# ieellee/uLLSAM

Measured on AMD Instinct MI355X. Metric: images/s end-to-end (ViT+LLM+mask) 1024^2, higher is better.
Workload: dtype bf16; 1 GPU; uLLSAM mask path (app.py:580-645): SAM ViT-H + InternLM2-7b-shaped prefill S=1081 + prompt encoder + mask decoder + x4 upsample/threshold, 1 point prompt/image, batch 4/GPU; batch_per_gpu=4, global_batch=4, seq_len=1081, vit_linears=bf16

## Files before the change

### ullsam_amd/csrc/norm.hip

```cpp
#include "common.h"

struct NormArgs {
    const void* in;
    void* out;
    const float* w;
    const float* b;
    long rows;
    int D;
    long in_stride, out_stride;
    float eps;
    int rms;
    int act;
    const float* post_scale;
    const float* post_shift;
};

template <typename TI, typename TO, int MAXV>
__global__ __launch_bounds__(256) void norm_kernel(NormArgs p) {
    const int lane = threadIdx.x & 63;
    const long row = (long)blockIdx.x * 4 + (threadIdx.x >> 6);
    if (row >= p.rows) return;
    const TI* x = reinterpret_cast<const TI*>(p.in) + row * p.in_stride;
    TO* y = reinterpret_cast<TO*>(p.out) + row * p.out_stride;
    const int nv = p.D >> 2;
    float4 v[MAXV];
    float s = 0.f;
#pragma unroll
    for (int i = 0; i < MAXV; ++i) {
        const int idx = i * 64 + lane;
        if (idx < nv) {
            v[i] = load4(x + idx * 4);
            s += (v[i].x + v[i].y) + (v[i].z + v[i].w);
        } else {
            v[i] = make_float4(0.f, 0.f, 0.f, 0.f);
        }
    }
    float mean = 0.f;
    if (!p.rms) mean = wave_sum(s) / (float)p.D;
    float ss = 0.f;
#pragma unroll
    for (int i = 0; i < MAXV; ++i) {
        const int idx = i * 64 + lane;
        if (idx < nv) {
            const float a = v[i].x - mean, b = v[i].y - mean, c = v[i].z - mean, d = v[i].w - mean;
            ss += (a * a + b * b) + (c * c + d * d);
        }
    }
    const float var = wave_sum(ss) / (float)p.D;
    const float rstd = p.rms ? rsqrtf(var + p.eps) : 1.0f / sqrtf(var + p.eps);
    const float ps = p.post_scale ? p.post_scale[0] : 1.f;
    const float pb = p.post_shift ? p.post_shift[0] : 0.f;
    const bool post = p.post_scale || p.post_shift;
#pragma unroll
    for (int i = 0; i < MAXV; ++i) {
        const int idx = i * 64 + lane;
        if (idx < nv) {
            float4 o = make_float4((v[i].x - mean) * rstd, (v[i].y - mean) * rstd, (v[i].z - mean) * rstd, (v[i].w - mean) * rstd);
            if (p.w) {
                const float4 w = *reinterpret_cast<const float4*>(p.w + idx * 4);
                o.x *= w.x; o.y *= w.y; o.z *= w.z; o.w *= w.w;
            }
            if (p.b) {
                const float4 b = *reinterpret_cast<const float4*>(p.b + idx * 4);
                o.x += b.x; o.y += b.y; o.z += b.z; o.w += b.w;
            }
            if (post) { o.x = o.x * ps + pb; o.y = o.y * ps + pb; o.z = o.z * ps + pb; o.w = o.w * ps + pb; }
            if (p.act == 1) { o.x = gelu_erf(o.x); o.y = gelu_erf(o.y); o.z = gelu_erf(o.z); o.w = gelu_erf(o.w); }
            store4(y + idx * 4, o);
        }
    }
}

template <typename TI, typename TO, int MAXV, int WPR = 4>
__global__ __launch_bounds__(256) void norm_block_kernel(NormArgs p) {
    __shared__ float red[2][4];
    constexpr int TPR = WPR * 64;
    const int tid = threadIdx.x, lane = tid & 63, wv = tid >> 6;
    const int sub = wv / WPR, t = tid - sub * TPR;
    const long row = (long)blockIdx.x * (4 / WPR) + sub;
    const bool live = row < p.rows;
    const TI* x = reinterpret_cast<const TI*>(p.in) + (live ? row : 0) * p.in_stride;
    TO* y = reinterpret_cast<TO*>(p.out) + (live ? row : 0) * p.out_stride;
    const int nv = p.D >> 2;
    float4 v[MAXV];
    float s = 0.f;
#pragma unroll
    for (int i = 0; i < MAXV; ++i) {
        const int idx = i * TPR + t;
        if (idx < nv && live) {
            v[i] = load4(x + idx * 4);
            s += (v[i].x + v[i].y) + (v[i].z + v[i].w);
        } else {
            v[i] = make_float4(0.f, 0.f, 0.f, 0.f);
        }
    }
    auto row_sum = [&](float part, int slot) -> float {
        part = wave_sum(part);
        if (lane == 0) red[slot][wv] = part;
        __syncthreads();
        float tot = red[slot][sub * WPR];
#pragma unroll
        for (int k = 1; k < WPR; ++k) tot += red[slot][sub * WPR + k];
        return tot;
    };
    float mean = 0.f;
    if (!p.rms) mean = row_sum(s, 0) / (float)p.D;
    float ss = 0.f;
#pragma unroll
    for (int i = 0; i < MAXV; ++i) {
        const int idx = i * TPR + t;
        if (idx < nv && live) {
            const float a = v[i].x - mean, b = v[i].y - mean, c = v[i].z - mean, d = v[i].w - mean;
            ss += (a * a + b * b) + (c * c + d * d);
        }
    }
    const float var = row_sum(ss, 1) / (float)p.D;
    const float rstd = p.rms ? rsqrtf(var + p.eps) : 1.0f / sqrtf(var + p.eps);
    const float ps = p.post_scale ? p.post_scale[0] : 1.f;
    const float pb = p.post_shift ? p.post_shift[0] : 0.f;
    const bool post = p.post_scale || p.post_shift;
    if (!live) return;
#pragma unroll
    for (int i = 0; i < MAXV; ++i) {
        const int idx = i * TPR + t;
        if (idx < nv) {
            float4 o = make_float4((v[i].x - mean) * rstd, (v[i].y - mean) * rstd, (v[i].z - mean) * rstd, (v[i].w - mean) * rstd);
            if (p.w) {
                const float4 w = *reinterpret_cast<const float4*>(p.w + idx * 4);
                o.x *= w.x; o.y *= w.y; o.z *= w.z; o.w *= w.w;
            }
            if (p.b) {
                const float4 b = *reinterpret_cast<const float4*>(p.b + idx * 4);
                o.x += b.x; o.y += b.y; o.z += b.z; o.w += b.w;
            }
            if (post) { o.x = o.x * ps + pb; o.y = o.y * ps + pb; o.z = o.z * ps + pb; o.w = o.w * ps + pb; }
            if (p.act == 1) { o.x = gelu_erf(o.x); o.y = gelu_erf(o.y); o.z = gelu_erf(o.z); o.w = gelu_erf(o.w); }
            store4(y + idx * 4, o);
        }
    }
}

template <typename TI, typename TO>
__global__ __launch_bounds__(256) void norm_narrow_kernel(NormArgs p) {
    const int lane = threadIdx.x & 63, sub = lane & 15;
    const long row = ((long)blockIdx.x * 4 + (threadIdx.x >> 6)) * 4 + (lane >> 4);
    const int nv = p.D >> 2;
    const bool on = row < p.rows && sub < nv;
    const TI* x = reinterpret_cast<const TI*>(p.in) + (on ? row : 0) * p.in_stride;
    float4 v = make_float4(0.f, 0.f, 0.f, 0.f);
    if (on) v = load4(x + sub * 4);
    float s = (v.x + v.y) + (v.z + v.w);
    float mean = 0.f;
    if (!p.rms) {
        for (int o = 8; o > 0; o >>= 1) s += __shfl_xor(s, o, 64);
        mean = s / (float)p.D;
    }
    float ss = 0.f;
    if (on) {
        const float a = v.x - mean, b = v.y - mean, c = v.z - mean, d = v.w - mean;
        ss = (a * a + b * b) + (c * c + d * d);
    }
    for (int o = 8; o > 0; o >>= 1) ss += __shfl_xor(ss, o, 64);
    const float var = ss / (float)p.D;
    const float rstd = p.rms ? rsqrtf(var + p.eps) : 1.0f / sqrtf(var + p.eps);
    if (!on) return;
    float4 o = make_float4((v.x - mean) * rstd, (v.y - mean) * rstd, (v.z - mean) * rstd, (v.w - mean) * rstd);
    if (p.w) {
        const float4 w = *reinterpret_cast<const float4*>(p.w + sub * 4);
        o.x *= w.x; o.y *= w.y; o.z *= w.z; o.w *= w.w;
    }
    if (p.b) {
        const float4 b = *reinterpret_cast<const float4*>(p.b + sub * 4);
        o.x += b.x; o.y += b.y; o.z += b.z; o.w += b.w;
    }
    if (p.post_scale || p.post_shift) {
        const float ps = p.post_scale ? p.post_scale[0] : 1.f, pb = p.post_shift ? p.post_shift[0] : 0.f;
        o.x = o.x * ps + pb; o.y = o.y * ps + pb; o.z = o.z * ps + pb; o.w = o.w * ps + pb;
    }
    if (p.act == 1) { o.x = gelu_erf(o.x); o.y = gelu_erf(o.y); o.z = gelu_erf(o.z); o.w = gelu_erf(o.w); }
    store4(reinterpret_cast<TO*>(p.out) + row * p.out_stride + sub * 4, o);
}

static int g_norm_lds = 0;
extern "C" int ullsam_set_norm_variant(int v) { g_norm_lds = v; return 0; }

template <typename TI, typename TO>
static int launch_norm(const NormArgs& a, hipStream_t s) {
    const dim3 grid((unsigned)((a.rows + 3) / 4)), block(256);
    const int nv = a.D / 4;
    if (nv <= 16 && a.rows >= 4096) {
        norm_narrow_kernel<TI, TO><<<dim3((unsigned)((a.rows + 15) / 16)), block, 0, s>>>(a);
        ULLSAM_LAUNCH_CHECK();
        return 0;
    }
    if (g_norm_lds == 0 && (a.rows >= 1024 || a.rows <= 64) && nv >= 512) {
        const dim3 g((unsigned)a.rows);
        if (nv <= 512) norm_block_kernel<TI, TO, 2><<<g, block, 0, s>>>(a);
        else norm_block_kernel<TI, TO, 4><<<g, block, 0, s>>>(a);
        ULLSAM_LAUNCH_CHECK();
        return 0;
    }
    const size_t lds = 0;
    if (nv <= 64) norm_kernel<TI, TO, 1><<<grid, block, lds, s>>>(a);
    else if (nv <= 256) norm_kernel<TI, TO, 4><<<grid, block, lds, s>>>(a);
    else if (nv <= 512) norm_kernel<TI, TO, 8><<<grid, block, lds, s>>>(a);
    else norm_kernel<TI, TO, 16><<<grid, block, lds, s>>>(a);
    ULLSAM_LAUNCH_CHECK();
    return 0;
}

template <typename TO>
__global__ __launch_bounds__(256) void norm_fanout_kernel(const float* __restrict__ in, long rows, int D, const float* __restrict__ w,
                                                          const float* __restrict__ b, float eps, float* __restrict__ out_f32,
                                                          TO* __restrict__ out_c, TO* __restrict__ out_c_pe,
                                                          const float* __restrict__ pe, long pe_rows) {
    const int lane = threadIdx.x & 63;
    const long row = (long)blockIdx.x * 4 + (threadIdx.x >> 6);
    if (row >= rows) return;
    const int nv = D >> 2;
    const bool on = lane < nv;
    float4 v = make_float4(0.f, 0.f, 0.f, 0.f);
    if (on) v = *reinterpret_cast<const float4*>(in + row * D + lane * 4);
    const float mean = wave_sum((v.x + v.y) + (v.z + v.w)) / (float)D;
    float ss = 0.f;
    if (on) {
        const float a = v.x - mean, bb = v.y - mean, c = v.z - mean, d = v.w - mean;
        ss = (a * a + bb * bb) + (c * c + d * d);
    }
    const float rstd = 1.0f / sqrtf(wave_sum(ss) / (float)D + eps);
    if (!on) return;
    float4 o = make_float4((v.x - mean) * rstd, (v.y - mean) * rstd, (v.z - mean) * rstd, (v.w - mean) * rstd);
    if (w) { const float4 t = *reinterpret_cast<const float4*>(w + lane * 4); o.x *= t.x; o.y *= t.y; o.z *= t.z; o.w *= t.w; }
    if (b) { const float4 t = *reinterpret_cast<const float4*>(b + lane * 4); o.x += t.x; o.y += t.y; o.z += t.z; o.w += t.w; }
    if (out_f32) *reinterpret_cast<float4*>(out_f32 + row * D + lane * 4) = o;
    if (out_c) store4(out_c + row * D + lane * 4, o);
    if (out_c_pe) {
        const float4 t = *reinterpret_cast<const float4*>(pe + (row % pe_rows) * D + lane * 4);
        store4(out_c_pe + row * D + lane * 4, make_float4(o.x + t.x, o.y + t.y, o.z + t.z, o.w + t.w));
    }
}

extern "C" int ullsam_norm_fanout(const float* in, long rows, int D, const float* w, const float* b, float eps, float* out_f32,
                                  void* out_c, void* out_c_pe, int c_dtype, const float* pe, long pe_rows, void* stream) {
    ULLSAM_CHECK(D % 4 == 0 && D > 0 && D <= 256, "norm_fanout: D=%d must be a multiple of 4 and <= 256", D);
    ULLSAM_CHECK(!out_c_pe || (pe && pe_rows > 0), "norm_fanout: out_c_pe needs pe");
    if (rows <= 0) return 0;
    hipStream_t s = reinterpret_cast<hipStream_t>(stream);
    const dim3 grid((unsigned)((rows + 3) / 4));
    if (c_dtype == 0) norm_fanout_kernel<float><<<grid, 256, 0, s>>>(in, rows, D, w, b, eps, out_f32, (float*)out_c, (float*)out_c_pe, pe, pe_rows);
    else norm_fanout_kernel<bf16><<<grid, 256, 0, s>>>(in, rows, D, w, b, eps, out_f32, (bf16*)out_c, (bf16*)out_c_pe, pe, pe_rows);
    ULLSAM_LAUNCH_CHECK();
    return 0;
}

extern "C" int ullsam_norm(const void* in, int in_dtype, long in_stride, void* out, int out_dtype, long out_stride,
                           const float* w, const float* b, long rows, int D, float eps, int rms, int act,
                           const float* post_scale, const float* post_shift, void* stream) {
    ULLSAM_CHECK(D % 4 == 0 && D > 0 && D <= 4096, "ullsam_norm: D=%d must be a multiple of 4 and <= 4096", D);
    ULLSAM_CHECK(rows >= 0, "ullsam_norm: bad rows");
    if (rows == 0) return 0;
    ULLSAM_CHECK(in_stride % 4 == 0 && out_stride % 4 == 0, "ullsam_norm: strides must be multiples of 4 elements");
    NormArgs a{in, out, w, rms ? nullptr : b, rows, D, in_stride, out_stride, eps, rms, act, post_scale, post_shift};
    hipStream_t s = reinterpret_cast<hipStream_t>(stream);
    if (in_dtype == 0 && out_dtype == 0) return launch_norm<float, float>(a, s);
    if (in_dtype == 0 && out_dtype == 1) return launch_norm<float, bf16>(a, s);
    if (in_dtype == 1 && out_dtype == 1) return launch_norm<bf16, bf16>(a, s);
    if (in_dtype == 1 && out_dtype == 0) return launch_norm<bf16, float>(a, s);
    ULLSAM_CHECK(false, "ullsam_norm: bad dtypes %d %d", in_dtype, out_dtype);
}

template <typename TI, int MAXV>
__global__ __launch_bounds__(256) void rows_fp8_kernel(const TI* __restrict__ in, long in_stride, unsigned char* __restrict__ out, long out_stride,
                                                      float* __restrict__ scale, const float* __restrict__ w, const float* __restrict__ b, long rows, int D,
                                                      float eps, int do_norm) {
    const int lane = threadIdx.x & 63;
    const long row = (long)blockIdx.x * 4 + (threadIdx.x >> 6);
    if (row >= rows) return;
    const TI* x = in + row * in_stride;
    const int nv = D >> 2;
    float4 v[MAXV];
    float s = 0.f;
#pragma unroll
    for (int i = 0; i < MAXV; ++i) {
        const int idx = i * 64 + lane;
        v[i] = idx < nv ? load4(x + idx * 4) : make_float4(0.f, 0.f, 0.f, 0.f);
        s += (v[i].x + v[i].y) + (v[i].z + v[i].w);
    }
    if (do_norm) {
        const float mean = wave_sum(s) / (float)D;
        float ss = 0.f;
#pragma unroll
        for (int i = 0; i < MAXV; ++i)
            if (i * 64 + lane < nv) {
                const float a = v[i].x - mean, bb = v[i].y - mean, c = v[i].z - mean, d = v[i].w - mean;
                ss += (a * a + bb * bb) + (c * c + d * d);
            }
        const float rstd = 1.0f / sqrtf(wave_sum(ss) / (float)D + eps);
#pragma unroll
        for (int i = 0; i < MAXV; ++i) {
            const int idx = i * 64 + lane;
            if (idx < nv) {
                const float4 g = *reinterpret_cast<const float4*>(w + idx * 4), be = *reinterpret_cast<const float4*>(b + idx * 4);
                v[i].x = (v[i].x - mean) * rstd * g.x + be.x; v[i].y = (v[i].y - mean) * rstd * g.y + be.y;
                v[i].z = (v[i].z - mean) * rstd * g.z + be.z; v[i].w = (v[i].w - mean) * rstd * g.w + be.w;
            }
        }
    }
    float amax = 0.f;
#pragma unroll
    for (int i = 0; i < MAXV; ++i) amax = fmaxf(amax, fmaxf(fmaxf(fabsf(v[i].x), fabsf(v[i].y)), fmaxf(fabsf(v[i].z), fabsf(v[i].w))));
    amax = wave_max(amax);
    const float sc = amax > 0.f ? amax * (1.0f / 448.0f) : 1.0f;
    const float inv = 1.0f / sc;
    if (lane == 0) scale[row] = sc;
    unsigned int* y = reinterpret_cast<unsigned int*>(out + row * out_stride);
#pragma unroll
    for (int i = 0; i < MAXV; ++i) {
        const int idx = i * 64 + lane;
        if (idx < nv) {
            const float q0 = fminf(fmaxf(v[i].x * inv, -448.f), 448.f), q1 = fminf(fmaxf(v[i].y * inv, -448.f), 448.f);
            const float q2 = fminf(fmaxf(v[i].z * inv, -448.f), 448.f), q3 = fminf(fmaxf(v[i].w * inv, -448.f), 448.f);
            int pk = __builtin_amdgcn_cvt_pk_fp8_f32(q0, q1, 0, false);
            pk = __builtin_amdgcn_cvt_pk_fp8_f32(q2, q3, pk, true);
            y[idx] = (unsigned int)pk;
        }
    }
}

extern "C" int ullsam_rows_fp8(const void* in, int in_dtype, long in_stride, void* out, long out_stride, float* scale, const float* w,
                               const float* b, long rows, int D, float eps, void* stream) {
    ULLSAM_CHECK(D % 4 == 0 && D <= 8192 && rows >= 0, "ullsam_rows_fp8: D=%d must be a multiple of 4, <= 8192", D);
    ULLSAM_CHECK((w == nullptr) == (b == nullptr), "ullsam_rows_fp8: weight and bias go together");
    ULLSAM_CHECK(out_stride % 4 == 0 && ((uintptr_t)out & 3) == 0, "ullsam_rows_fp8: output rows must be 4-byte aligned");
    if (rows == 0) return 0;
    hipStream_t s = reinterpret_cast<hipStream_t>(stream);
    const dim3 grid((unsigned)((rows + 3) / 4));
    const int nv = D / 4, maxv = (nv + 63) / 64;
    const int dn = w != nullptr;
#define ULLSAM_RF8(TI, MV) rows_fp8_kernel<TI, MV><<<grid, 256, 0, s>>>(reinterpret_cast<const TI*>(in), in_stride, reinterpret_cast<unsigned char*>(out), out_stride, scale, w, b, rows, D, eps, dn)
    if (in_dtype == ULLSAM_DT_F32) {
        if (maxv <= 4) ULLSAM_RF8(float, 4); else if (maxv <= 8) ULLSAM_RF8(float, 8); else if (maxv <= 16) ULLSAM_RF8(float, 16); else ULLSAM_RF8(float, 32);
    } else {
        if (maxv <= 4) ULLSAM_RF8(bf16, 4); else if (maxv <= 8) ULLSAM_RF8(bf16, 8); else if (maxv <= 16) ULLSAM_RF8(bf16, 16); else ULLSAM_RF8(bf16, 32);
    }
#undef ULLSAM_RF8
    ULLSAM_LAUNCH_CHECK();
    return 0;
}

template <typename TI>
__global__ __launch_bounds__(256) void rows_fp8_pow2_kernel(const TI* __restrict__ in, long in_stride, unsigned char* __restrict__ out, long out_stride,
                                                           float* __restrict__ scale, long rows, int D) {
    const int lane = threadIdx.x & 63;
    const long row = (long)blockIdx.x * 4 + (threadIdx.x >> 6);
    if (row >= rows) return;
    const TI* x = in + row * in_stride;
    const int nv = D >> 2;
    float amax = 0.f;
    for (int idx = lane; idx < nv; idx += 64) {
        const float4 v = load4(x + idx * 4);
        amax = fmaxf(amax, fmaxf(fmaxf(fabsf(v.x), fabsf(v.y)), fmaxf(fabsf(v.z), fabsf(v.w))));
    }
    amax = wave_max(amax);
    float sc = 1.0f, inv = 1.0f;
    if (amax > 0.f) {
        int e;
        const float f = frexpf(amax, &e);
        const int s = max((f <= 0.875f ? e - 9 : e - 8), -126);
        sc = ldexpf(1.0f, s);
        inv = ldexpf(1.0f, -s);
    }
    if (lane == 0) scale[row] = sc;
    unsigned int* y = reinterpret_cast<unsigned int*>(out + row * out_stride);
    for (int idx = lane; idx < nv; idx += 64) {
        const float4 v = load4(x + idx * 4);
        const float q0 = fminf(fmaxf(v.x * inv, -448.f), 448.f), q1 = fminf(fmaxf(v.y * inv, -448.f), 448.f);
        const float q2 = fminf(fmaxf(v.z * inv, -448.f), 448.f), q3 = fminf(fmaxf(v.w * inv, -448.f), 448.f);
        int pk = __builtin_amdgcn_cvt_pk_fp8_f32(q0, q1, 0, false);
        pk = __builtin_amdgcn_cvt_pk_fp8_f32(q2, q3, pk, true);
        y[idx] = (unsigned int)pk;
    }
}

extern "C" int ullsam_rows_fp8_pow2(const void* in, int in_dtype, long in_stride, void* out, long out_stride, float* scale, long rows, int D,
                                    void* stream) {
    ULLSAM_CHECK(in_dtype == ULLSAM_DT_F32 || in_dtype == ULLSAM_DT_BF16, "ullsam_rows_fp8_pow2: bad dtype %d", in_dtype);
    ULLSAM_CHECK(D > 0 && D % 4 == 0 && rows >= 0 && rows <= 4l * 0x7fffffff, "ullsam_rows_fp8_pow2: D=%d must be a positive multiple of 4", D);
    ULLSAM_CHECK(in_stride >= D && in_stride % 4 == 0 && ((uintptr_t)in & (in_dtype == ULLSAM_DT_F32 ? 15 : 7)) == 0, "ullsam_rows_fp8_pow2: input rows must be aligned groups of 4 elements");
    ULLSAM_CHECK(out_stride >= D && out_stride % 4 == 0 && ((uintptr_t)out & 3) == 0, "ullsam_rows_fp8_pow2: output rows must be 4-byte aligned");
    ULLSAM_CHECK(in && out && scale, "ullsam_rows_fp8_pow2: null argument");
    if (rows == 0) return 0;
    hipStream_t s = reinterpret_cast<hipStream_t>(stream);
    const dim3 grid((unsigned)((rows + 3) / 4));
    if (in_dtype == ULLSAM_DT_F32) rows_fp8_pow2_kernel<float><<<grid, 256, 0, s>>>(reinterpret_cast<const float*>(in), in_stride, reinterpret_cast<unsigned char*>(out), out_stride, scale, rows, D);
    else rows_fp8_pow2_kernel<bf16><<<grid, 256, 0, s>>>(reinterpret_cast<const bf16*>(in), in_stride, reinterpret_cast<unsigned char*>(out), out_stride, scale, rows, D);
    ULLSAM_LAUNCH_CHECK();
    return 0;
}
```

Baseline: 54.03 images/s.

## Add persistent double-buffered streaming layernorm kernel for fp32-to-bf16 rows

Adds a persistent grid-stride norm kernel for fp32-in, bf16-out rows at common widths (1280, 2048, 3072, 4096). It keeps weights and bias in registers, prefetches the next row while reducing the current one, and pairs lanes with DPP swaps to issue 16-byte stores. The grid is capped at a few workgroups per CU. The goal is to hide load latency and cut launch and tail overhead for the ViT and LLM norms, at the cost of more register use, a changed reduction order, and new variant-flag encoding.

```diff
diff --git a/ullsam_amd/csrc/norm.hip b/ullsam_amd/csrc/norm.hip
--- a/ullsam_amd/csrc/norm.hip
+++ b/ullsam_amd/csrc/norm.hip
@@ -1,4 +1,5 @@
 #include "common.h"
+#include <type_traits>
 
 struct NormArgs {
     const void* in;
@@ -181,19 +182,164 @@
     store4(reinterpret_cast<TO*>(p.out) + row * p.out_stride + sub * 4, o);
 }
 
-static int g_norm_lds = 0;
-extern "C" int ullsam_set_norm_variant(int v) { g_norm_lds = v; return 0; }
+typedef unsigned int u32x4 __attribute__((ext_vector_type(4)));
+
+template <bool NT> __device__ __forceinline__ f32x4 load_row4(const float* p) {
+    if (NT) return __builtin_nontemporal_load(reinterpret_cast<const f32x4*>(p));
+    return *reinterpret_cast<const f32x4*>(p);
+}
+__device__ __forceinline__ float centred_sumsq(f32x4 v, float mean) {
+#pragma clang fp contract(off)
+    const float a = v.x - mean, b = v.y - mean, c = v.z - mean, d = v.w - mean;
+    return __builtin_fmaf(a, a, b * b) + __builtin_fmaf(c, c, d * d);
+}
+__device__ __forceinline__ uint2v norm_affine_bf16(f32x4 v, float mean, float rstd, float4 w, float4 b, bool has_w, bool has_b) {
+#pragma clang fp contract(off)
+    float4 o = make_float4((v.x - mean) * rstd, (v.y - mean) * rstd, (v.z - mean) * rstd, (v.w - mean) * rstd);
+    if (has_w) { o.x *= w.x; o.y *= w.y; o.z *= w.z; o.w *= w.w; }
+    if (has_b) { o.x += b.x; o.y += b.y; o.z += b.z; o.w += b.w; }
+    bf16x4_t h;
+    h[0] = (bf16)o.x; h[1] = (bf16)o.y; h[2] = (bf16)o.z; h[3] = (bf16)o.w;
+    return __builtin_bit_cast(uint2v, h);
+}
+__device__ __forceinline__ unsigned int lane_xor1(unsigned int v) { return (unsigned int)__builtin_amdgcn_mov_dpp((int)v, 0xB1, 0xF, 0xF, true); }
+
+template <int NV, int WPR, bool NT>
+__global__ __launch_bounds__(256) void norm_stream_kernel(NormArgs p) {
+    __shared__ float red[4][4];
+    constexpr int TPR = WPR * 64;
+    const int tid = threadIdx.x, lane = tid & 63, wv = tid >> 6;
+    const int t = WPR == 1 ? lane : tid;
+    long row = WPR == 1 ? (long)blockIdx.x * 4 + __builtin_amdgcn_readfirstlane(wv) : (long)blockIdx.x;
+    const long stride = WPR == 1 ? (long)gridDim.x * 4 : (long)gridDim.x;
+    const float* xin = reinterpret_cast<const float*>(p.in);
+    bf16* yout = reinterpret_cast<bf16*>(p.out);
+    const bool has_w = p.w != nullptr, has_b = p.b != nullptr;
+    float4 w[NV], b[NV];
+#pragma unroll
+    for (int i = 0; i < NV; ++i) {
+        w[i] = has_w ? *reinterpret_cast<const float4*>(p.w + (i * TPR + t) * 4) : make_float4(0.f, 0.f, 0.f, 0.f);
+        b[i] = has_b ? *reinterpret_cast<const float4*>(p.b + (i * TPR + t) * 4) : make_float4(0.f, 0.f, 0.f, 0.f);
+    }
+    auto row_sum = [&](float part, int slot) -> float {
+        part = wave_sum(part);
+        if (WPR == 1) return part;
+        if (lane == 0) red[slot][wv] = part;
+        __syncthreads();
+        float tot = red[slot][0];
+#pragma unroll
+        for (int k = 1; k < 4; ++k) tot += red[slot][k];
+        return tot;
+    };
+    if (row >= p.rows) return;
+    auto issue = [&](f32x4 (&v)[NV], long r, int spread) {
+        const float* x = xin + r * p.in_stride;
+#pragma unroll
+        for (int i = 0; i < NV; ++i) v[i] = load_row4<NT>(x + (i * TPR + t) * 4 * spread);
+    };
+    int left = (int)((p.rows - row + stride - 1) / stride);
+    auto next = [&]() -> int {
+        int more = __builtin_amdgcn_readfirstlane((int)(left > 1));
+        asm volatile("" : "+s"(more));
+        --left;
+        return more;
+    };
+    auto finish = [&](const f32x4 (&v)[NV], long r, int slot) {
+        float s = 0.f;
+#pragma unroll
+        for (int i = 0; i < NV; ++i) s += (v[i].x + v[i].y) + (v[i].z + v[i].w);
+        float mean = 0.f;
+        if (!p.rms) mean = row_sum(s, slot) / (float)p.D;
+        float ss = 0.f;
+#pragma unroll
+        for (int i = 0; i < NV; ++i) ss += centred_sumsq(v[i], mean);
+        const float var = row_sum(ss, slot + 1) / (float)p.D;
+        const float rstd = p.rms ? rsqrtf(var + p.eps) : 1.0f / sqrtf(var + p.eps);
+        bf16* y = yout + r * p.out_stride;
+        const bool odd = t & 1;
+#pragma unroll
+        for (int i = 0; i + 1 < NV; i += 2) {
+            const uint2v A = norm_affine_bf16(v[i], mean, rstd, w[i], b[i], has_w, has_b);
+            const uint2v B = norm_affine_bf16(v[i + 1], mean, rstd, w[i + 1], b[i + 1], has_w, has_b);
+            const uint2v give = odd ? A : B;
+            const uint2v got = {lane_xor1(give.x), lane_xor1(give.y)};
+            const int idx = odd ? (i + 1) * TPR + t - 1 : i * TPR + t;
+            const u32x4 o = odd ? u32x4{got.x, got.y, B.x, B.y} : u32x4{A.x, A.y, got.x, got.y};
+            *reinterpret_cast<u32x4*>(y + idx * 4) = o;
+        }
+        if (NV & 1) {
+            const uint2v A = norm_affine_bf16(v[NV - 1], mean, rstd, w[NV - 1], b[NV - 1], has_w, has_b);
+            *reinterpret_cast<uint2v*>(y + ((NV - 1) * TPR + t) * 4) = A;
+        }
+    };
+    f32x4 va[NV], vb[NV];
+    issue(va, row, 1);
+    int more = next();
+    issue(vb, row + stride * more, more);
+    finish(va, row, 0);
+    if (!more) return;
+    row += stride;
+    more = next();
+    issue(va, row + stride * more, more);
+    finish(vb, row, 2);
+    if (!more) return;
+    row += stride;
+    for (;;) {
+        more = next();
+        issue(vb, row + stride * more, more);
+        finish(va, row, 0);
+        if (!more) break;
+        row += stride;
+        more = next();
+        issue(va, row + stride * more, more);
+        finish(vb, row, 2);
+        if (!more) break;
+        row += stride;
+    }
+}
+
+static int g_norm_variant = 0;
+extern "C" int ullsam_set_norm_variant(int v) { g_norm_variant = v; return 0; }
+constexpr int NORM_STREAM_WG_PER_CU = 4;
+
+static int norm_cu_count() {
+    static PerDeviceOnce cu_once; static int n_cu = 256;
+    if (cu_once.first()) { int dev = 0; hipDeviceProp_t pr; if (hipGetDevice(&dev) == hipSuccess && hipGetDeviceProperties(&pr, dev) == hipSuccess && pr.multiProcessorCount > 0) n_cu = pr.multiProcessorCount; }
+    return n_cu;
+}
+
+template <int NV, int WPR>
+static int launch_norm_stream(const NormArgs& a, hipStream_t s) {
+    const int per_cu = (g_norm_variant >> 8) & 0xff;
+    const long cap = (long)norm_cu_count() * (per_cu ? per_cu : NORM_STREAM_WG_PER_CU);
+    const long want = WPR == 1 ? (a.rows + 3) / 4 : a.rows;
+    const dim3 grid((unsigned)(want < cap ? want : cap));
+    if (g_norm_variant & 0x10000) norm_stream_kernel<NV, WPR, true><<<grid, 256, 0, s>>>(a);
+    else norm_stream_kernel<NV, WPR, false><<<grid, 256, 0, s>>>(a);
+    ULLSAM_LAUNCH_CHECK();
+    return 0;
+}
 
 template <typename TI, typename TO>
 static int launch_norm(const NormArgs& a, hipStream_t s) {
     const dim3 grid((unsigned)((a.rows + 3) / 4)), block(256);
     const int nv = a.D / 4;
+    const int g_norm_lds = g_norm_variant & 0xff;
+    if constexpr (std::is_same<TI, float>::value && std::is_same<TO, bf16>::value) {
+        if (g_norm_lds == 0 && a.rows >= 1024 && a.act == 0 && !a.post_scale && !a.post_shift && a.in_stride >= a.D && a.out_stride >= a.D &&
+            a.out_stride % 8 == 0 && ((uintptr_t)a.in & 15) == 0 && ((uintptr_t)a.out & 15) == 0) {
+            if (a.D == 1280) return launch_norm_stream<5, 1>(a, s);
+            if (a.D == 2048) return launch_norm_stream<2, 4>(a, s);
+            if (a.D == 3072) return launch_norm_stream<3, 4>(a, s);
+            if (a.D == 4096) return launch_norm_stream<4, 4>(a, s);
+        }
+    }
     if (nv <= 16 && a.rows >= 4096) {
         norm_narrow_kernel<TI, TO><<<dim3((unsigned)((a.rows + 15) / 16)), block, 0, s>>>(a);
         ULLSAM_LAUNCH_CHECK();
         return 0;
     }
-    if (g_norm_lds == 0 && (a.rows >= 1024 || a.rows <= 64) && nv >= 512) {
+    if (g_norm_lds != 1 && (a.rows >= 1024 || a.rows <= 64) && nv >= 512) {
         const dim3 g((unsigned)a.rows);
         if (nv <= 512) norm_block_kernel<TI, TO, 2><<<g, block, 0, s>>>(a);
         else norm_block_kernel<TI, TO, 4><<<g, block, 0, s>>>(a);
```

Result: no change. 54.45 images/s, median of 6 (+0.8%).
